# JelleAalbers/blueice

Hardware: AMD Instinct MI355X
Metric: likelihood evals/sec (and GB/s vs HBM peak), 4-src 5^3-anchor 100^3-bin model (higher is better)
Workload: dtype f64; 1 GPU; C2: 4 sources, 3 shape params (5^3 anchors), 100^3 bins; step = one batched call (one kernel launch) of 8 independent dense evaluations, each against its own dataset, in grid cells that share no anchor (no byte re-used), tensor replicated per GPU; device=gfx950:sramecc+:xnack-, gather=none (one process), backend_requested=rccl, backend_explicit=False, gather_kind=none (one process)

## Files before the change

blueice_amd/csrc/bi_context.h:

```cpp
#pragma once

struct bi_ctx;

constexpr int kThreads = 256;
constexpr int kBinsPerThread = 2;
constexpr int kTile = kThreads * kBinsPerThread;
constexpr int kMaxDim = 8;
constexpr int kMaxG = 16;

inline thread_local std::string g_create_error;

struct DevBuf {
    void* p = nullptr;
    size_t bytes = 0;
    struct bi_ctx* owner = nullptr;
    bool view = false;
};

struct bi_plan {
    int64_t P = 0;
    struct Class {
        int G = 0;
        int64_t n_items = 0;
        int nbx = 0;
// ... 42 lines not shown
    hipDeviceProp_t prop{};
    std::string err;

    bool model_ready = false, model_open = false;
    int d = 0, S = 0;
    int64_t B = 0, Bp = 0, A = 0;
    std::vector<int> n_anchor;
    std::vector<std::vector<double>> grid;
    std::vector<int64_t> astride;
    std::vector<int> eff_axes;
    int bb_source = -1;
    std::vector<int32_t> allow_neg;
    DevBuf ps, nm, nm_tot;
    std::vector<double> h_mus;
    std::vector<double> h_nm_tot;
    std::vector<char> anchor_set;

    int space_k = 0;
    std::vector<int32_t> space_n_edges;
    DevBuf space_edges;

    bool unbinned = false;
    double outlier = 0.0;
    bool ps_finite = true;
    bool data_ready = false;
    bool dense_counts = false;
    int64_t T = 0;
    DevBuf counts, lgsum;
    std::vector<double> h_lgsum;

    std::vector<double> h_rowsum;
    std::vector<double> h_rowmin;
    bool ps_nonneg = false;

    bool csr_ready = false, compact_ready = false;
    bool compact_sorted = false;
    DevBuf nz_idx, nz_n, nz_off, ps_c, cnt_c;
    DevBuf tm_entries, tm_off;
    int64_t nz_tile_epoch = -1;
    bool tm_ok = false;
    DevBuf tmm_entries, tmm_off;
    int64_t tmm_epoch = -1;
    bool tmm_ok = false;
    int tmm_width = 4;
    int64_t toy_points_pp = 0;
    int64_t toy_points_lanes = 0;
    int64_t toy_points_overlap = 0;
    hipStream_t stream2 = nullptr;
    hipEvent_t tp_ev[7] = {nullptr, nullptr, nullptr, nullptr, nullptr, nullptr, nullptr};
    int64_t n_toy_points_passes = 0;
    int64_t dot_tiled = 1;
    int64_t score_sorted = 1;
    DevBuf ev_perm;
    bool ev_sorted = false;
    int64_t toy_fast_call = 7;
    DevBuf toy_blocks_done;
    bool toy_blocks_done_zeroed = false;
    unsigned long long toy_seq = 0;
    int64_t n_toy_polled = 0;
    int64_t dot_entry16 = 1;
    int tm_width = 4;
    int64_t dot_blocks_per_cu = 0;
    int64_t dot_lanes = 0;
    int64_t toy_events = 1;
    int64_t last_toy_method = 0;
    std::vector<int64_t> h_nz_off;
    std::vector<int64_t> h_c_off, h_cnt_off;
    std::vector<int64_t> h_c_np;
    std::vector<double> h_Tz;

    DevBuf slot_dev, slot_partial, slot_pflags, slot_counter;
    DevBuf mail, mail_flags;
    void* pack_host = nullptr;
    void* bounce_host = nullptr;
    size_t pack_host_bytes = 0;
    DevBuf pack_dev;
    void* plan_host = nullptr;
    unsigned long long plan_seq = 0;
    void* slot_host = nullptr;
    size_t slot_host_bytes = 0;
    unsigned long long slot_seq = 0;
    int64_t single_ns[3] = {0, 0, 0};
    int64_t single_calls = 0;
    int pending = 0;
    unsigned long long pending_seq = 0;
    double pending_ll = 0.0;
    int32_t pending_status = 0;

    DevBuf pt_grid, pt_mus, pt_coff, pt_allow, pt_c_off, pt_cnt_off, pt_c_np, pt_Tz, pt_rowsum, pt_rowmin, pt_nm_tot;
    int64_t plan_tables_epoch = -1;
    bool plan_tables_sparse = false;
    int64_t n_valid_launches = 0;
    int64_t n_scan_launches = 0;
    int64_t last_scan_nslots = 0, last_scan_resident = 0, last_valid_nslots = 0;
    int64_t grad_mfma = 1;
    int64_t grad_mfma_min = 2048;
    int64_t grad_slices = 0;
    int64_t n_grad_mfma_launches = 0;
    int64_t scan_xcd = 1;
    int64_t scan_share_slow = 1;
    int64_t plan_count_sort = 1;
    int64_t plan_tables = 1;
    int64_t scan_chunk = 1;
    int64_t scan_waves_per_cu = 0;
    int64_t keep_rows = -1;
    int64_t last_single_cell = -1, last_single_ds = -1;
    int64_t poll_result = 1;
    int64_t tile_chunks = 8;
    int64_t scan_min_items = 4;
    int64_t toy_offset = 0;
    int64_t scan_cb = 0;
    int64_t bb_exact = 2;
    int64_t n_bb_exact = 0;
    int64_t scan_sparse_max_items = (int64_t)1 << 40;
    int64_t scan_split = 1;
    int64_t sparse_at_upload = 1;
    int64_t scan_mfma = 1;
    int64_t scan_pow = 1;
    DevBuf ps_sorted, cnt_sorted;
    int64_t sorted_epoch = -1;
    bool sorted_ok = false;
    int64_t n_sorted_scans = 0;
    int64_t mail_timeout_ms = 2000;
    int64_t debug_skip_post = -1, debug_late_post = -1;
    int64_t n_mail_resets = 0;
    std::vector<void*> user_allocs;
    int64_t bb_max_group = 8;
    int64_t scan_bb = 1;
    int64_t scan_bb_min = 64;
    int64_t n_bb_scan_launches = 0;
    int64_t device_plan_min = 512;

    DevBuf sim_coords, sim_source;
    int sim_k = 0;
    int64_t sim_n = -1;

    DevBuf scratch, scratch2, logmu;

    std::vector<DevBuf> cache;
    size_t cache_bytes = 0;

    int64_t epoch = 0;

    int64_t blocks_per_cu = 8;
    int64_t max_group = kMaxG;
    int64_t xcd_affine = 1;
    int64_t fuse_max_blocks = (int64_t)1 << 20;
    int64_t single_blocks_per_cu = 4;
    int64_t fuse_finish = 1;
    int64_t single_kernel = 1;
    int64_t nt_loads = 2;
    int64_t sparse = 1;
    int64_t compact_budget = (int64_t)16 << 30;

    bool profiling = false;
    std::vector<std::pair<hipEvent_t, hipEvent_t>> ev_pool;
    size_t ev_used = 0;
    int64_t prof_launches = 0;
    double prof_ms = 0.0;
};

namespace {

int fail(bi_ctx* c, int code, const char* fmt, ...) {
    char buf[512];
    va_list ap;
    va_start(ap, fmt);
    vsnprintf(buf, sizeof buf, fmt, ap);
    va_end(ap);
    if (c) c->err = buf; else g_create_error = buf;
    return code;
}

#define HIP_TRY(c, expr)                                                                          \
    do {                                                                                          \
        hipError_t e_ = (expr);                                                                   \
        if (e_ != hipSuccess)                                                                     \
            return fail((c), BI_ERR_HIP, "%s failed: %s (%s:%d)", #expr, hipGetErrorString(e_), __FILE__, __LINE__); \
    } while (0)

constexpr size_t kCacheMaxBuf = (size_t)1 << 30;
constexpr size_t kCacheMaxTotal = (size_t)4 << 30;
constexpr size_t kCacheMaxEntries = 256;

void dev_free(DevBuf& b) {
    if (b.p && !b.view) {
        bi_ctx* c = b.owner;
        if (c && b.bytes <= kCacheMaxBuf && c->cache.size() < kCacheMaxEntries && c->cache_bytes + b.bytes <= kCacheMaxTotal) {
            c->cache.push_back(b);
            c->cache_bytes += b.bytes;
        } else {
            (void)hipFree(b.p);
        }
    }
    b.p = nullptr;
    b.bytes = 0;
    b.view = false;
}

void drop_recycle_cache(bi_ctx* c) {
    (void)hipGetLastError();
    for (auto& q : c->cache) (void)hipFree(q.p);
    c->cache.clear();
    c->cache_bytes = 0;
}

int dev_alloc(bi_ctx* c, DevBuf& b, size_t bytes) {
    if (b.p && b.bytes >= bytes) return BI_OK;
    if (b.p) dev_free(b);
    if (bytes == 0) bytes = 16;
    if (bytes <= kCacheMaxBuf) {
        size_t best = (size_t)-1;
        for (size_t i = 0; i < c->cache.size(); ++i)
            if (c->cache[i].bytes >= bytes && c->cache[i].bytes <= 4 * bytes + 4096 &&
                (best == (size_t)-1 || c->cache[i].bytes < c->cache[best].bytes))
                best = i;
        if (best != (size_t)-1) {
            b = c->cache[best];
            c->cache_bytes -= b.bytes;
            c->cache[best] = c->cache.back();
            c->cache.pop_back();
            return BI_OK;
        }
    }
    hipError_t e = hipMalloc(&b.p, bytes);
    if (e != hipSuccess) {
        drop_recycle_cache(c);
        e = hipMalloc(&b.p, bytes);
    }
    if (e != hipSuccess) {
        b.p = nullptr;
        return fail(c, BI_ERR_NOMEM, "hipMalloc(%zu bytes) failed: %s", bytes, hipGetErrorString(e));
    }
    b.bytes = bytes;
    b.owner = c;
    return BI_OK;
}

template <class T>
int dev_upload(bi_ctx* c, DevBuf& b, const std::vector<T>& h) {
    int rc = dev_alloc(c, b, h.size() * sizeof(T));
    if (rc) return rc;
    if (!h.empty()) HIP_TRY(c, hipMemcpyAsync(b.p, h.data(), h.size() * sizeof(T), hipMemcpyHostToDevice, c->stream));
    return BI_OK;
}

struct PackedUpload {
    std::vector<size_t> off;
    size_t in_bytes = 0, out_off = 0;
    char* dev_base = nullptr;
    char* host_base = nullptr;
    template <typename T>
    const T* dev(size_t i) const { return reinterpret_cast<const T*>(dev_base + off[i]); }
    void* host_out() const { return host_base + out_off; }
};

inline int packed_upload(bi_ctx* c, const std::vector<std::pair<const void*, size_t>>& parts, size_t out_bytes, PackedUpload& pu,
                         DevBuf* slab = nullptr) {
    pu.off.clear();
    size_t total = 0;
    for (const auto& part : parts) {
        pu.off.push_back(total);
        total += (part.second + 63) / 64 * 64;
    }
    pu.in_bytes = total;
    pu.out_off = total;
    const size_t need = total + (out_bytes + 63) / 64 * 64 + 64;
    if (c->pack_host_bytes < need) {
        if (c->pack_host) { HIP_TRY(c, hipStreamSynchronize(c->stream)); HIP_TRY(c, hipHostFree(c->pack_host)); c->pack_host = nullptr; c->pack_host_bytes = 0; }
        const size_t grow = std::max<size_t>(2 * need, 65536);
        HIP_TRY(c, hipHostMalloc(&c->pack_host, grow, hipHostMallocDefault));
        c->pack_host_bytes = grow;
    }
    DevBuf& dst = slab ? *slab : c->pack_dev;
    int rc = dev_alloc(c, dst, std::max<size_t>(total, 64));
    if (rc) return rc;
    pu.host_base = (char*)c->pack_host;
    pu.dev_base = (char*)dst.p;
    for (size_t i = 0; i < parts.size(); ++i)
        if (parts[i].second) memcpy(pu.host_base + pu.off[i], parts[i].first, parts[i].second);
    if (total) HIP_TRY(c, hipMemcpyAsync(pu.dev_base, pu.host_base, total, hipMemcpyHostToDevice, c->stream));
    return BI_OK;
}

void free_plan_buffers(bi_plan* p) {
    for (auto& k : p->classes) {
        dev_free(k.rowoff); dev_free(k.coef); dev_free(k.aux); dev_free(k.item_cnt); dev_free(k.item_tiles);
        dev_free(k.perm); dev_free(k.slot_lg); dev_free(k.partial); dev_free(k.pflags); dev_free(k.rowoff_full);
    }
    dev_free(p->bad_idx); dev_free(p->nan_idx); dev_free(p->out); dev_free(p->status); dev_free(p->grp_first); dev_free(p->grp_items);
    dev_free(p->slab); dev_free(p->bad); dev_free(p->sorted_idx); dev_free(p->keep_z); dev_free(p->keep_rs);
}

}
```

blueice_amd/csrc/bi_k_misc.h:

```cpp
#pragma once

namespace {

__global__ void k_selftest_log(const double* __restrict__ x, int64_t n, double* __restrict__ out) {
    log_table_load();
    const int64_t i = (int64_t)blockIdx.x * blockDim.x + threadIdx.x;
    if (i < n) out[i] = bin_log(x[i]);
}

template <bool NT>
__global__ __launch_bounds__(kThreads) void k_read_sum(const double* __restrict__ p, int64_t n2, double* __restrict__ sink) {
    double s = 0.0;
    const int64_t stride = (int64_t)gridDim.x * kThreads;
    int64_t i = (int64_t)blockIdx.x * kThreads + threadIdx.x;
    for (; i + 7 * stride < n2; i += 8 * stride) {
        double2 v[8];
#pragma unroll
        for (int u = 0; u < 8; ++u) v[u] = stream_load<NT>(p + 2 * (i + u * stride));
#pragma unroll
        for (int u = 0; u < 8; ++u) s += v[u].x + v[u].y;
    }
    for (; i < n2; i += stride) s += p[2 * i] + p[2 * i + 1];
    if (s == 0.123456789) sink[0] = s;
}
// ... 275 lines not shown
    const double* __restrict__ r = rows + (int64_t)blockIdx.x * Bp;
    double s = 0.0, mn = __builtin_inf(), bad = 0.0;
    {
        double s4[4] = {0.0, 0.0, 0.0, 0.0};
        int64_t b = threadIdx.x;
        for (; b + 3 * kThreads < B; b += 4 * kThreads) {
            double v[4];
#pragma unroll
            for (int k = 0; k < 4; ++k) v[k] = r[b + k * kThreads];
#pragma unroll
            for (int k = 0; k < 4; ++k) {
                s4[k] += v[k];
                mn = fmin(mn, v[k]);
                if (!(fabs(v[k]) < __builtin_inf())) bad = 1.0;
            }
        }
        for (; b < B; b += kThreads) {
            const double v = r[b];
            s4[0] += v;
            mn = fmin(mn, v);
            if (!(fabs(v) < __builtin_inf())) bad = 1.0;
        }
        s = (s4[0] + s4[1]) + (s4[2] + s4[3]);
    }
    __shared__ double sh[3][kThreads / 64];
    s = wave_sum(s);
    bad = wave_sum(bad);
#pragma unroll
    for (int off = 32; off > 0; off >>= 1) mn = fmin(mn, __shfl_down(mn, off, 64));
    if ((threadIdx.x & 63) == 0) { sh[0][threadIdx.x >> 6] = s; sh[1][threadIdx.x >> 6] = mn; sh[2][threadIdx.x >> 6] = bad; }
    __syncthreads();
    if (threadIdx.x == 0) {
        double t = sh[0][0], m = sh[1][0], f = sh[2][0];
        for (int w = 1; w < kThreads / 64; ++w) { t += sh[0][w]; m = fmin(m, sh[1][w]); f += sh[2][w]; }
        out[(int64_t)blockIdx.x * 3 + 0] = t;
        out[(int64_t)blockIdx.x * 3 + 1] = m;
        out[(int64_t)blockIdx.x * 3 + 2] = f;
    }
}

constexpr int kNzPerThread = 8;
constexpr int kNzChunk = kThreads * kNzPerThread;

__device__ __forceinline__ bool is_nz(double n) { return n != 0.0; }

__global__ __launch_bounds__(kThreads) void k_nz_count(const double* __restrict__ counts, int64_t B, int64_t Bp,
                                                       int32_t* __restrict__ cnt, int nchunks) {
    const double* __restrict__ c = counts + (int64_t)blockIdx.y * Bp;
    const int64_t b0 = (int64_t)blockIdx.x * kNzChunk + threadIdx.x * kNzPerThread;
    int k = 0;
#pragma unroll
    for (int j = 0; j < kNzPerThread; ++j)
        if (b0 + j < B && is_nz(c[b0 + j])) ++k;
    __shared__ int sh[kThreads / 64];
#pragma unroll
    for (int off = 32; off > 0; off >>= 1) k += __shfl_down(k, off, 64);
    if ((threadIdx.x & 63) == 0) sh[threadIdx.x >> 6] = k;
    __syncthreads();
    if (threadIdx.x == 0) cnt[(int64_t)blockIdx.y * nchunks + blockIdx.x] = sh[0] + sh[1] + sh[2] + sh[3];
}

__global__ __launch_bounds__(kThreads) void k_nz_scatter(const double* __restrict__ counts, int64_t B, int64_t Bp,
                                                         const int64_t* __restrict__ chunk_off, int nchunks,
                                                         int32_t* __restrict__ nz_idx, double* __restrict__ nz_n) {
    const double* __restrict__ c = counts + (int64_t)blockIdx.y * Bp;
    const int64_t b0 = (int64_t)blockIdx.x * kNzChunk + threadIdx.x * kNzPerThread;
    double v[kNzPerThread];
    int k = 0;
#pragma unroll
    for (int j = 0; j < kNzPerThread; ++j) {
        v[j] = (b0 + j < B) ? c[b0 + j] : 0.0;
        if (is_nz(v[j])) ++k;
    }
    const int lane = threadIdx.x & 63, wave = threadIdx.x >> 6;
    int incl = k;
#pragma unroll
    for (int off = 1; off < 64; off <<= 1) {
        const int t = __shfl_up(incl, off, 64);
        if (lane >= off) incl += t;
    }
    __shared__ int sh[kThreads / 64];
    if (lane == 63) sh[wave] = incl;
    __syncthreads();
    int base = 0;
    for (int w = 0; w < wave; ++w) base += sh[w];
    int64_t pos = chunk_off[(int64_t)blockIdx.y * nchunks + blockIdx.x] + base + incl - k;
#pragma unroll
    for (int j = 0; j < kNzPerThread; ++j)
        if (is_nz(v[j])) {
            nz_idx[pos] = (int32_t)(b0 + j);
            nz_n[pos] = v[j];
            ++pos;
        }
}

__global__ __launch_bounds__(kThreads) void k_gather_rows(const double* __restrict__ rows, int64_t Bp,
                                                          const int32_t* __restrict__ idx, int64_t nnz, int64_t np,
                                                          double* __restrict__ out) {
    const int64_t j = (int64_t)blockIdx.x * kThreads + threadIdx.x;
    if (j >= np) return;
    const int64_t row = blockIdx.y;
    out[row * np + j] = j < nnz ? rows[row * Bp + idx[j]] : 0.0;
}

__global__ void k_pad_copy(const double* __restrict__ src, int64_t n, int64_t np, double* __restrict__ dst) {
    const int64_t j = (int64_t)blockIdx.x * blockDim.x + threadIdx.x;
    if (j < np) dst[j] = j < n ? src[j] : 0.0;
}

__global__ __launch_bounds__(kThreads) void k_dataset_dot_csr(const int32_t* __restrict__ nz_idx,
                                                              const double* __restrict__ nz_n,
                                                              const int64_t* __restrict__ nz_off,
                                                              const double* __restrict__ logmu, int64_t t0,
                                                              double* __restrict__ partial) {
    const int64_t t = t0 + blockIdx.x;
    const int64_t lo = nz_off[t], hi = nz_off[t + 1];
    double s = 0.0;
    for (int64_t j = lo + threadIdx.x; j < hi; j += kThreads) {
        const double n = nz_n[j];
        double term = n * logmu[nz_idx[j]];
        if (n != n) term = __builtin_nan("");
        else if (n < 0.0 || n != floor(n)) term = -__builtin_inf();
        s += term;
    }
    __shared__ double sh[kThreads / 64];
    s = wave_sum(s);
    if ((threadIdx.x & 63) == 0) sh[threadIdx.x >> 6] = s;
    __syncthreads();
    if (threadIdx.x == 0) {
        double r = sh[0];
        for (int w = 1; w < kThreads / 64; ++w) r += sh[w];
        partial[blockIdx.x] = r;
    }
}

constexpr int kDotTile = 8192;

__global__ __launch_bounds__(kThreads) void k_csr_tile_offsets(const int32_t* __restrict__ nz_idx, const int64_t* __restrict__ nz_off,
                                                               int n_tl, int32_t* __restrict__ tile_off ,
                                                               int tile_shift ) {
    const int64_t t = blockIdx.x;
    const int64_t lo = nz_off[t], hi = nz_off[t + 1];
    int32_t* __restrict__ dst = tile_off + t * (n_tl + 1);
    if (hi == lo) {
        for (int tl = threadIdx.x; tl <= n_tl; tl += kThreads) dst[tl] = 0;
        return;
    }
    for (int64_t j = lo + threadIdx.x; j < hi; j += kThreads) {
        const int cur = nz_idx[j] >> tile_shift;
        const int prev = j > lo ? nz_idx[j - 1] >> tile_shift : -1;
        for (int tl = prev + 1; tl <= cur; ++tl) dst[tl] = (int32_t)(j - lo);
        if (j == hi - 1)
            for (int tl = cur + 1; tl <= n_tl; ++tl) dst[tl] = (int32_t)(hi - lo);
    }
}

__device__ __forceinline__ double row16_sum(double v) {
#define BI_ROR_ADD(N)                                                                                              \
    do {                                                                                                           \
        const unsigned long long u = __double_as_longlong(v);                                                      \
        const unsigned lo = __builtin_amdgcn_update_dpp(0, (int)(unsigned)u, 0x120 + N, 0xF, 0xF, true);           \
        const unsigned hi = __builtin_amdgcn_update_dpp(0, (int)(unsigned)(u >> 32), 0x120 + N, 0xF, 0xF, true);   \
        v += __longlong_as_double(((unsigned long long)hi << 32) | lo);                                            \
    } while (0)
    BI_ROR_ADD(8);
    BI_ROR_ADD(4);
    BI_ROR_ADD(2);
    BI_ROR_ADD(1);
#undef BI_ROR_ADD
    return v;
}

constexpr uint32_t kTmPadEntry = (uint32_t)kDotTile << 3;
__global__ void k_tm_counts(const int32_t* __restrict__ tile_off, int64_t T, int n_tl, int64_t* __restrict__ cnt ,
                            int group ) {
    const int64_t i = (int64_t)blockIdx.x * blockDim.x + threadIdx.x;
    if (i > (int64_t)n_tl * T) return;
    if (i == (int64_t)n_tl * T) { cnt[i] = 0; return; }
    const int64_t tl = i / T, t = i % T;
    const int32_t* __restrict__ o = tile_off + t * (n_tl + 1) + tl;
    cnt[i] = (o[1] - o[0] + group - 1) & ~(group - 1);
}

template <typename ENTRY>
__global__ __launch_bounds__(kThreads) void k_tm_scatter(const int32_t* __restrict__ nz_idx, const double* __restrict__ nz_n,
                                                         const int64_t* __restrict__ nz_off, const int32_t* __restrict__ tile_off,
                                                         int64_t T, int n_tl, const int64_t* __restrict__ tm_off,
                                                         ENTRY* __restrict__ tm_entries, int* __restrict__ bad, int tile_shift) {
    const int64_t t = blockIdx.x;
    const int64_t lo = nz_off[t], hi = nz_off[t + 1];
    const int32_t* __restrict__ o = tile_off + t * (n_tl + 1);
    bool any_bad = false;
    for (int64_t j = lo + threadIdx.x; j < hi; j += kThreads) {
        const int idx = nz_idx[j];
        const double n = nz_n[j];
        const int tl = idx >> tile_shift;
        if constexpr (sizeof(ENTRY) == 2) {
            if (!(n >= 1.0 && n <= 7.0 && n == floor(n))) any_bad = true;
            tm_entries[tm_off[(int64_t)tl * T + t] + (j - lo - o[tl])] = (ENTRY)(((uint32_t)(idx - (tl << tile_shift)) << 3) | ((uint32_t)n & 7u));
        } else {
            if (!(n >= 1.0 && n < 32768.0 && n == floor(n))) any_bad = true;
            tm_entries[tm_off[(int64_t)tl * T + t] + (j - lo - o[tl])] = ((uint32_t)(idx - (tl << tile_shift)) << 3) | ((uint32_t)n << 17);
        }
    }
    if (any_bad) atomicOr(bad, 1);
}

typedef uint32_t bi_uint4 __attribute__((ext_vector_type(4)));
constexpr int kDotThreads = 1024;
#ifndef BI_DOT_DEPTH
#define BI_DOT_DEPTH 2
#endif
constexpr int kDotPad = 64 * 2 + 16;

template <int L>
__device__ __forceinline__ double row_group_sum(double v) {
#define BI_DPP_ADD(CTRL)                                                                                           \
    do {                                                                                                           \
        const unsigned long long u = __double_as_longlong(v);                                                      \
        const unsigned lo = __builtin_amdgcn_update_dpp(0, (int)(unsigned)u, CTRL, 0xF, 0xF, true);                \
        const unsigned hi = __builtin_amdgcn_update_dpp(0, (int)(unsigned)(u >> 32), CTRL, 0xF, 0xF, true);        \
        v += __longlong_as_double(((unsigned long long)hi << 32) | lo);                                            \
    } while (0)
    if constexpr (L == 16) {
        BI_DPP_ADD(0x120 + 8);
        BI_DPP_ADD(0x120 + 4);
        BI_DPP_ADD(0x120 + 2);
        BI_DPP_ADD(0x120 + 1);
    } else if constexpr (L == 8) {
        BI_DPP_ADD(0x141);
        BI_DPP_ADD(0xB1);
        BI_DPP_ADD(0x4E);
    } else if constexpr (L == 4) {
        BI_DPP_ADD(0xB1);
        BI_DPP_ADD(0x4E);
    } else {
        static_assert(L == 2, "groups of 2, 4, 8 or 16 lanes");
        BI_DPP_ADD(0xB1);
    }
#undef BI_DPP_ADD
    return v;
}

template <int L, int AHEAD, int W = 4>
__global__ __launch_bounds__(kDotThreads) void k_dataset_dot_tiled(const void* __restrict__ tm_entries_v,
                                                                   const int64_t* __restrict__ tm_off, int64_t T, int n_tl,
                                                                   const double* __restrict__ logmu, int64_t B, int64_t t0,
                                                                   int64_t n, double* __restrict__ partial ) {
    typedef typename std::conditional<W == 2, uint16_t, uint32_t>::type entry_t;
    constexpr int EPL = 16 / W;
    static_assert(EPL * L * AHEAD + 16 <= kDotPad, "the lists' padding must cover the read-ahead");
    const entry_t* __restrict__ tm_entries = static_cast<const entry_t*>(tm_entries_v);
    __shared__ double s_mu[kDotTile + 1];
    const int tl = blockIdx.x;
    const int64_t bin0 = (int64_t)tl * kDotTile;
    const int row = threadIdx.x / L, gl = threadIdx.x % L;
    const int per = (int)((n + gridDim.y - 1) / gridDim.y);
    const int c0u = (int)blockIdx.y * per, c1 = min((int)n, c0u + per);
    const int c0 = min(c0u, (int)n - 1);
    const int64_t* __restrict__ off = tm_off + (int64_t)tl * T + t0;
    const int64_t base = off[c0];
    const entry_t* __restrict__ ent = tm_entries + base;
    const uint32_t* __restrict__ off32 = reinterpret_cast<const uint32_t*>(off);
    const uint32_t base32 = (uint32_t)base;
    constexpr int kStep = kDotThreads / L, kAhead = AHEAD, kDepth = BI_DOT_DEPTH, kRing = 2 * (kDepth + 1);
    const int q_last = max(c0, c1 - 1);
    auto load_offsets = [&](int q, uint32_t& ra, uint32_t& rb) {
        const int qc = min(q, q_last);
        ra = off32[2 * qc];
        rb = off32[2 * qc + 2];
    };
    auto load_entries = [&](uint32_t ra, bi_uint4 (&e)[kAhead]) {
        const entry_t* __restrict__ p = ent + (int)(ra - base32) + EPL * gl;
#pragma unroll
        for (int k = 0; k < kAhead; ++k) __builtin_memcpy(&e[k], p + EPL * L * k, 16);
    };
    bi_uint4 E[kDepth + 1][kAhead];
    uint32_t RA[kRing], RB[kRing];
    const int q0 = c0 + row;
#pragma unroll
    for (int u = 0; u < 2 * kDepth; ++u) load_offsets(q0 + u * kStep, RA[u], RB[u]);
    {
        double v[kDotTile / kDotThreads];
#pragma unroll
        for (int k = 0; k < kDotTile / kDotThreads; ++k) v[k] = logmu[min(bin0 + threadIdx.x + k * kDotThreads, B - 1)];
#pragma unroll
        for (int k = 0; k < kDotTile / kDotThreads; ++k)
            s_mu[threadIdx.x + k * kDotThreads] = bin0 + threadIdx.x + k * kDotThreads < B ? v[k] : 0.0;
        if (threadIdx.x == 0) s_mu[kDotTile] = 0.0;
    }
#pragma unroll
    for (int u = 0; u < kDepth; ++u) load_entries(RA[u], E[u]);
    __syncthreads();
    if (c0u >= c1) return;
    const int n_iter = (c1 - c0 + kStep - 1) / kStep;
    for (int it = 0; it < n_iter; it += kRing) {
#pragma unroll
        for (int u = 0; u < kRing; ++u) {
            if (it + u < n_iter) {
                const int q = q0 + (it + u) * kStep;
                load_offsets(q + 2 * kDepth * kStep, RA[(u + 2 * kDepth) % kRing], RB[(u + 2 * kDepth) % kRing]);
                load_entries(RA[(u + kDepth) % kRing], E[(u + kDepth) % (kDepth + 1)]);
                __builtin_amdgcn_sched_barrier(0);
                const bi_uint4 (&e)[kAhead] = E[u % (kDepth + 1)];
                const int a = (int)(RA[u % kRing] - base32), b = (int)(RB[u % kRing] - base32);
                const int len = b - a - EPL * gl;
// ... 784 lines not shown
```

blueice_amd/csrc/bi_params.h:

```cpp
#pragma once

namespace {

enum : int { kParamRead = 1, kParamWrite = 2, kParamRW = 3 };

struct ParamDef {
    const char* name;
    int access;
    int64_t (*get)(bi_ctx*);
    int (*set)(bi_ctx*, int64_t);
};

#define BI_P_GET(expr) [](bi_ctx* c) -> int64_t { return (int64_t)(expr); }
#define BI_P_SET(stmt) [](bi_ctx* c, int64_t v) -> int { stmt; return BI_OK; }
#define BI_P_RANGE(lo, hi, field, what)                                                                           \
    [](bi_ctx* c, int64_t v) -> int {                                                                             \
        if (v < (lo) || v > (hi)) return fail(c, BI_ERR_INVALID, what);                                           \
        c->field = v;                                                                                             \
        return BI_OK;                                                                                             \
    }
#define BI_P_FLAG(field) BI_P_SET(c->field = v ? 1 : 0)
#define BI_P_RO(nm, expr) {nm, kParamRead, BI_P_GET(expr), nullptr}

const ParamDef kParams[] = {
    {"sparse", kParamRW, BI_P_GET(c->sparse), BI_P_RANGE(0, 2, sparse, "sparse: 0 = off, 1 = auto, 2 = whenever exact")},
    {"max_group", kParamRW, BI_P_GET(c->max_group),
     [](bi_ctx* c, int64_t v) -> int {
         if (v < 1 || v > kMaxG || (v & (v - 1))) return fail(c, BI_ERR_INVALID, "max_group must be a power of two in [1,%d]", kMaxG);
         c->max_group = v;
         return BI_OK;
     }},
    {"bb_max_group", kParamRW, BI_P_GET(c->bb_max_group), BI_P_SET(c->bb_max_group = v >= 16 ? 16 : (v >= 8 ? 8 : (v >= 4 ? 4 : (v >= 2 ? 2 : 1))))},
    {"blocks_per_cu", kParamRW, BI_P_GET(c->blocks_per_cu), BI_P_RANGE(1, 32, blocks_per_cu, "blocks_per_cu in [1,32]")},
    {"nt_loads", kParamRW, BI_P_GET(c->nt_loads), BI_P_RANGE(0, 2, nt_loads, "nt_loads: 0 = never, 1 = always, 2 = auto")},
    {"tile_chunks", kParamRW, BI_P_GET(c->tile_chunks), BI_P_SET(c->tile_chunks = v < 1 ? 1 : v)},
    {"single_kernel", kParamRW, BI_P_GET(c->single_kernel), BI_P_FLAG(single_kernel)},
    {"fuse_max_blocks", kParamRW, BI_P_GET(c->fuse_max_blocks), BI_P_SET(c->fuse_max_blocks = v)},
    {"single_blocks_per_cu", kParamRW, BI_P_GET(c->single_blocks_per_cu),
     BI_P_RANGE(1, 32, single_blocks_per_cu, "single_blocks_per_cu in [1,32]")},
    {"fuse_finish", kParamRW, BI_P_GET(c->fuse_finish), BI_P_FLAG(fuse_finish)},
    {"keep_rows", kParamRW, BI_P_GET(c->keep_rows), BI_P_SET(c->keep_rows = v < 0 ? -1 : v)},
    {"poll_result", kParamRW, BI_P_GET(c->poll_result), BI_P_FLAG(poll_result)},
    {"xcd_affine", kParamRW, BI_P_GET(c->xcd_affine), BI_P_FLAG(xcd_affine)},
    {"device_plan_min", kParamRW, BI_P_GET(c->device_plan_min), BI_P_SET(c->device_plan_min = v)},
    {"scan_mfma", kParamRW, BI_P_GET(c->scan_mfma), BI_P_FLAG(scan_mfma)},
    {"scan_min_items", kParamRW, BI_P_GET(c->scan_min_items), BI_P_SET(c->scan_min_items = v < 1 ? 1 : v)},
    {"scan_cb", kParamRW, BI_P_GET(c->scan_cb), BI_P_SET(c->scan_cb = (v == 2 || v == 4) ? v : 0)},
    {"scan_waves_per_cu", kParamRW, BI_P_GET(c->scan_waves_per_cu), BI_P_SET(c->scan_waves_per_cu = v < 0 ? 0 : v)},
    {"host_threads", kParamRW, [](bi_ctx*) -> int64_t { return host_threads(); },
     [](bi_ctx* c, int64_t v) -> int { if (v < 0 || v > 256) return fail(c, BI_ERR_INVALID, "host_threads in [0, 256] (0 = by the process's affinity, at most 16)"); host_threads_setting().store((int)v); return BI_OK; }},
    {"toy_points_pp", kParamRW, BI_P_GET(c->toy_points_pp),
     [](bi_ctx* c, int64_t v) -> int {
         if (v != 0 && v != 1 && v != 2 && v != 4) return fail(c, BI_ERR_INVALID, "toy_points_pp: 0 = by the batch, 1 = point by point, 2 or 4 points per pass");
         c->toy_points_pp = v;
         return BI_OK;
     }},
    {"toy_points_overlap", kParamRW, BI_P_GET(c->toy_points_overlap), BI_P_FLAG(toy_points_overlap)},
    {"toy_points_lanes", kParamRW, BI_P_GET(c->toy_points_lanes),
     [](bi_ctx* c, int64_t v) -> int {
         if (v != 0 && v != 2 && v != 4 && v != 8) return fail(c, BI_ERR_INVALID, "toy_points_lanes: 0 = default, or 2 / 4 / 8");
         c->toy_points_lanes = v;
         return BI_OK;
     }},
    {"grad_mfma", kParamRW, BI_P_GET(c->grad_mfma), BI_P_FLAG(grad_mfma)},
    {"grad_mfma_min", kParamRW, BI_P_GET(c->grad_mfma_min), BI_P_RANGE(1, (int64_t)1 << 40, grad_mfma_min, "grad_mfma_min >= 1")},
    {"grad_slices", kParamRW, BI_P_GET(c->grad_slices), BI_P_RANGE(0, 4096, grad_slices, "grad_slices in [0, 4096]")},
    {"scan_xcd", kParamRW, BI_P_GET(c->scan_xcd), BI_P_RANGE(0, 2, scan_xcd, "scan_xcd: 0 launch order, 1 contiguous ranges, 2 one XCD per group")},
    {"scan_share_slow", kParamRW, BI_P_GET(c->scan_share_slow), BI_P_FLAG(scan_share_slow)},
    {"scan_chunk", kParamRW, BI_P_GET(c->scan_chunk), BI_P_FLAG(scan_chunk)},
    {"plan_tables", kParamRW, BI_P_GET(c->plan_tables), BI_P_FLAG(plan_tables)},
    {"plan_count_sort", kParamRW, BI_P_GET(c->plan_count_sort), BI_P_FLAG(plan_count_sort)},
    {"scan_bb", kParamRW, BI_P_GET(c->scan_bb), BI_P_FLAG(scan_bb)},
    {"scan_bb_min", kParamRW, BI_P_GET(c->scan_bb_min), BI_P_RANGE(1, (int64_t)1 << 40, scan_bb_min, "scan_bb_min >= 1")},
    {"scan_sparse_max_items", kParamRW, BI_P_GET(c->scan_sparse_max_items), BI_P_SET(c->scan_sparse_max_items = v < 0 ? 0 : v)},
    {"scan_split", kParamRW, BI_P_GET(c->scan_split), BI_P_FLAG(scan_split)},
    {"scan_pow", kParamRW, BI_P_GET(c->scan_pow), BI_P_SET(c->scan_pow = v ? 1 : 0; c->sorted_epoch = -1)},
    {"bb_exact", kParamRW, BI_P_GET(c->bb_exact), BI_P_RANGE(0, 2, bb_exact, "bb_exact: 0 never, 1 always, 2 auto")},
    {"toy_events", kParamRW, BI_P_GET(c->toy_events), BI_P_FLAG(toy_events)},
    {"dot_tiled", kParamRW, BI_P_GET(c->dot_tiled), BI_P_FLAG(dot_tiled)},
    {"score_sorted", kParamRW, BI_P_GET(c->score_sorted), BI_P_FLAG(score_sorted)},
    {"toy_fast_call", kParamRW, BI_P_GET(c->toy_fast_call), BI_P_RANGE(0, 7, toy_fast_call, "toy_fast_call: bits 1 | 2 | 4")},
    {"dot_entry16", kParamRW, BI_P_GET(c->dot_entry16), [](bi_ctx* c, int64_t v) -> int { c->dot_entry16 = v ? 1 : 0; c->nz_tile_epoch = -1; c->tmm_epoch = -1; return BI_OK; }},
    {"dot_blocks_per_cu", kParamRW, BI_P_GET(c->dot_blocks_per_cu), BI_P_RANGE(0, 16, dot_blocks_per_cu, "dot_blocks_per_cu in [0, 16]")},
    {"dot_lanes", kParamRW, BI_P_GET(c->dot_lanes), BI_P_SET(c->dot_lanes = (v == 16 || v == 8 || v == 4) ? v : 0)},
    {"compact_budget", kParamRW, BI_P_GET(c->compact_budget), BI_P_SET(c->compact_budget = v)},
    {"toy_offset", kParamRW, BI_P_GET(c->toy_offset), BI_P_RANGE(0, INT64_MAX, toy_offset, "toy_offset >= 0")},
    {"mail_timeout_ms", kParamRW, BI_P_GET(c->mail_timeout_ms),
     BI_P_RANGE(1, 60000, mail_timeout_ms, "mail_timeout_ms in [1, 60000]")},
    {"single_timing_reset", kParamWrite, nullptr,
     BI_P_SET(c->single_ns[0] = c->single_ns[1] = c->single_ns[2] = 0; c->single_calls = 0; (void)v)},
    {"drop_recycle_cache", kParamWrite, nullptr, BI_P_SET((void)hipSetDevice(c->device); (void)hipStreamSynchronize(c->stream); drop_recycle_cache(c); (void)v)},
    {"debug_skip_post", kParamWrite, nullptr, BI_P_SET(c->debug_skip_post = v < 0 ? -1 : v)},
    {"debug_late_post", kParamWrite, nullptr, BI_P_SET(c->debug_late_post = v < 0 ? -1 : v)},
    BI_P_RO("tile_bins", kTile),
    BI_P_RO("padded_bins", c->Bp),
    BI_P_RO("n_scan_launches", c->n_scan_launches),
    BI_P_RO("n_toy_polled", c->n_toy_polled),
    BI_P_RO("n_toy_points_passes", c->n_toy_points_passes),
    BI_P_RO("n_bb_scan_launches", c->n_bb_scan_launches),
    BI_P_RO("tmm_entry_bytes", c->tmm_ok ? c->tmm_width : 0),
    BI_P_RO("tm_entry_bytes", c->tm_width),
    BI_P_RO("events_sorted", c->ev_sorted ? 1 : 0),
    BI_P_RO("n_grad_mfma_launches", c->n_grad_mfma_launches),
    BI_P_RO("n_valid_launches", c->n_valid_launches),
    BI_P_RO("n_sorted_scans", c->n_sorted_scans),
    BI_P_RO("n_bb_exact", c->n_bb_exact),
    BI_P_RO("n_mail_resets", c->n_mail_resets),
    BI_P_RO("csr_ready", (c->csr_ready && (c->sparse_at_upload != 0 || !c->dense_counts)) ? 1 : 0),
    BI_P_RO("compact_ready", (c->compact_ready && c->ps_nonneg && (c->sparse_at_upload != 0 || !c->dense_counts)) ? 1 : 0),
    BI_P_RO("split_ready", (c->compact_ready && c->dense_counts) ? 1 : 0),
    BI_P_RO("ps_nonneg", c->ps_nonneg ? 1 : 0),
    BI_P_RO("compact_sorted", (c->compact_ready && c->compact_sorted) ? 1 : 0),
    BI_P_RO("nnz_total", c->csr_ready ? c->h_nz_off.back() : -1),
    BI_P_RO("last_scan_nslots", c->last_scan_nslots),
    BI_P_RO("last_valid_nslots", c->last_valid_nslots),
    BI_P_RO("last_scan_resident", c->last_scan_resident),
    BI_P_RO("last_toy_method", c->last_toy_method),
    BI_P_RO("single_calls", c->single_calls),
    BI_P_RO("single_ns_host", c->single_ns[0]),
    BI_P_RO("single_ns_launch", c->single_ns[1]),
    BI_P_RO("single_ns_wait", c->single_ns[2]),
    BI_P_RO("user_allocations", (int64_t)c->user_allocs.size()),
    BI_P_RO("recycle_cache_bytes", (int64_t)c->cache_bytes),
};

#undef BI_P_GET
#undef BI_P_SET
#undef BI_P_RANGE
#undef BI_P_FLAG
#undef BI_P_RO

const ParamDef* find_param(const char* name) {
    for (const ParamDef& p : kParams)
        if (!strcmp(p.name, name)) return &p;
    return nullptr;
}

}
```

blueice_amd/csrc/bi_sparse.h:

```cpp
#pragma once

#include <rocprim/rocprim.hpp>

namespace {

int build_compact_templates(bi_ctx* c) {
    c->compact_ready = false;
    const int64_t T = c->T, Bp = c->Bp;
    int rc;
    hipError_t e;
    if (c->bb_source >= 0 || !c->ps_finite) return BI_OK;
    const int64_t rows = c->A * c->S;
    c->h_c_np.assign((size_t)T, 0);
    c->h_c_off.assign((size_t)T, 0);
    c->h_cnt_off.assign((size_t)T, 0);
    int64_t tot_ps = 0, tot_cnt = 0;
    for (int64_t t = 0; t < T; ++t) {
        const int64_t nnz = c->h_nz_off[(size_t)t + 1] - c->h_nz_off[(size_t)t];
        const int64_t np = std::max<int64_t>(kTile, (nnz + kTile - 1) / kTile * kTile);
        c->h_c_np[(size_t)t] = np;
        c->h_c_off[(size_t)t] = tot_ps;
        c->h_cnt_off[(size_t)t] = tot_cnt;
        tot_ps += rows * np;
        tot_cnt += np;
    }
    if ((tot_ps + tot_cnt) * (int64_t)sizeof(double) > c->compact_budget) return BI_OK;
    auto roomy = [&](DevBuf& b, size_t bytes) { return b.p && b.bytes >= bytes ? BI_OK : dev_alloc(c, b, bytes + bytes / 8); };
    if ((rc = roomy(c->ps_c, (size_t)tot_ps * sizeof(double))) || (rc = roomy(c->cnt_c, (size_t)tot_cnt * sizeof(double))) ||
        (rc = dev_alloc(c, c->scratch, (size_t)T * rows * sizeof(double))))
        return rc;
    c->h_Tz.assign((size_t)T * rows, 0.0);
    std::vector<double> tnz((size_t)T * rows);
    c->compact_sorted = false;
    const bool sort_by_count = c->scan_pow && T <= 64;
    DevBuf d_sidx, d_sn, d_tmp;
    auto drop = [&]() { dev_free(d_sidx); dev_free(d_sn); dev_free(d_tmp); };
    for (int64_t t = 0; t < T; ++t) {
        const int64_t lo = c->h_nz_off[(size_t)t], nnz = c->h_nz_off[(size_t)t + 1] - lo, np = c->h_c_np[(size_t)t];
        double* dst = (double*)c->ps_c.p + c->h_c_off[(size_t)t];
        const int32_t* idx = (const int32_t*)c->nz_idx.p + lo;
        const double* cnt = (const double*)c->nz_n.p + lo;
        if (sort_by_count && nnz > 1) {
            size_t tmp_bytes = 0;
            (void)prim_sort_pairs(nullptr, tmp_bytes, (const double*)nullptr, (double*)nullptr, (const int32_t*)nullptr,
                                            (int32_t*)nullptr, (size_t)nnz, 0u, 64u, c->stream);
            if ((rc = dev_alloc(c, d_sidx, (size_t)nnz * sizeof(int32_t))) || (rc = dev_alloc(c, d_sn, (size_t)nnz * sizeof(double))) ||
                (rc = dev_alloc(c, d_tmp, std::max<size_t>(tmp_bytes, 256)))) { drop(); return rc; }
            size_t tb = d_tmp.bytes;
            e = prim_sort_pairs(d_tmp.p, tb, cnt, (double*)d_sn.p, idx, (int32_t*)d_sidx.p, (size_t)nnz, 0u, 64u, c->stream);
            if (e != hipSuccess) { drop(); return fail(c, BI_ERR_HIP, "template compaction (sort by count): %s", hipGetErrorString(e)); }
            idx = (const int32_t*)d_sidx.p;
            cnt = (const double*)d_sn.p;
        }
        hipLaunchKernelGGL(k_gather_rows, dim3((unsigned)((np + kThreads - 1) / kThreads), (unsigned)rows), dim3(kThreads), 0,
                           c->stream, (const double*)c->ps.p, Bp, idx, nnz, np, dst);
        hipLaunchKernelGGL(k_pad_copy, dim3((unsigned)((np + 255) / 256)), dim3(256), 0, c->stream,
                           cnt, nnz, np, (double*)c->cnt_c.p + c->h_cnt_off[(size_t)t]);
        hipLaunchKernelGGL(k_row_total, dim3((unsigned)rows), dim3(kThreads), 0, c->stream, (const double*)dst, np, np,
                           (double*)c->scratch.p + t * rows);
        e = hipGetLastError();
        if (e != hipSuccess) { (void)hipStreamSynchronize(c->stream); drop(); return fail(c, BI_ERR_HIP, "template compaction: %s", hipGetErrorString(e)); }
    }
    e = hipMemcpyAsync(tnz.data(), c->scratch.p, tnz.size() * sizeof(double), hipMemcpyDeviceToHost, c->stream);
    if (e == hipSuccess) e = hipStreamSynchronize(c->stream);
    else (void)hipStreamSynchronize(c->stream);
    drop();
    if (e != hipSuccess) return fail(c, BI_ERR_HIP, "template compaction: %s", hipGetErrorString(e));
    for (int64_t t = 0; t < T; ++t)
        for (int64_t r = 0; r < rows; ++r) c->h_Tz[(size_t)(t * rows + r)] = c->h_rowsum[(size_t)r] - tnz[(size_t)(t * rows + r)];
    c->compact_sorted = sort_by_count;
    c->compact_ready = true;
    return BI_OK;
}

int build_sparse_forms(bi_ctx* c) {
    c->csr_ready = c->compact_ready = false;
    const int64_t T = c->T, B = c->B, Bp = c->Bp;
    const int nchunks = (int)((B + kNzChunk - 1) / kNzChunk);
    int rc;
    DevBuf d_cnt, d_off;
    auto cleanup = [&]() { dev_free(d_cnt); dev_free(d_off); };
    if ((rc = dev_alloc(c, d_cnt, (size_t)T * nchunks * sizeof(int32_t)))) return rc;
    const int64_t tchunk = 32768;
    for (int64_t t0 = 0; t0 < T; t0 += tchunk) {
        const int64_t n = std::min(tchunk, T - t0);
        hipLaunchKernelGGL(k_nz_count, dim3((unsigned)nchunks, (unsigned)n), dim3(kThreads), 0, c->stream,
                           (const double*)c->counts.p + t0 * Bp, B, Bp, (int32_t*)d_cnt.p + t0 * nchunks, nchunks);
    }
    std::vector<int32_t> h_cnt((size_t)T * nchunks);
    hipError_t e = hipGetLastError();
    if (e == hipSuccess) e = hipMemcpyAsync(h_cnt.data(), d_cnt.p, h_cnt.size() * sizeof(int32_t), hipMemcpyDeviceToHost, c->stream);
    if (e == hipSuccess) e = hipStreamSynchronize(c->stream);
    if (e != hipSuccess) { cleanup(); return fail(c, BI_ERR_HIP, "non-empty-bin count: %s", hipGetErrorString(e)); }
    std::vector<int64_t> h_off(h_cnt.size());
    c->h_nz_off.assign((size_t)T + 1, 0);
    int64_t run = 0;
    for (int64_t t = 0; t < T; ++t) {
        c->h_nz_off[(size_t)t] = run;
        for (int k = 0; k < nchunks; ++k) { h_off[(size_t)t * nchunks + k] = run; run += h_cnt[(size_t)t * nchunks + k]; }
    }
    c->h_nz_off[(size_t)T] = run;
    c->sparse_at_upload = c->sparse;
    if (run > T * B / 4 && c->sparse != 2) { cleanup(); return BI_OK; }
    if ((rc = dev_upload(c, d_off, h_off)) || (rc = dev_alloc(c, c->nz_idx, (size_t)std::max<int64_t>(run, 1) * sizeof(int32_t))) ||
        (rc = dev_alloc(c, c->nz_n, (size_t)std::max<int64_t>(run, 1) * sizeof(double))) || (rc = dev_upload(c, c->nz_off, c->h_nz_off))) {
        cleanup();
        return rc;
    }
    for (int64_t t0 = 0; t0 < T; t0 += tchunk) {
        const int64_t n = std::min(tchunk, T - t0);
        hipLaunchKernelGGL(k_nz_scatter, dim3((unsigned)nchunks, (unsigned)n), dim3(kThreads), 0, c->stream,
                           (const double*)c->counts.p + t0 * Bp, B, Bp, (const int64_t*)d_off.p + t0 * nchunks, nchunks,
                           (int32_t*)c->nz_idx.p, (double*)c->nz_n.p);
    }
    e = hipGetLastError();
    if (e == hipSuccess) e = hipStreamSynchronize(c->stream);
    cleanup();
    if (e != hipSuccess) return fail(c, BI_ERR_HIP, "non-empty-bin scatter: %s", hipGetErrorString(e));
    c->csr_ready = true;

    return build_compact_templates(c);
}

}
```

Measured before the change: 26110 evals/s.

## Batch sparse template compaction across all templates with tiled gather kernels

Replaces the per-template loop of compaction launches with a batched path. Offsets are tiled per template, then one gather kernel stages each row's bin tile in shared memory and scatters the non-empty bins to every template's compacted output. Batched kernels then do padding copy and row totals. This targets setup cost from many small launches; the per-evaluation likelihood kernels are unchanged. It adds complexity and a flag to fall back to the old path.

```diff
diff --git a/blueice_amd/csrc/bi_context.h b/blueice_amd/csrc/bi_context.h
--- a/blueice_amd/csrc/bi_context.h
+++ b/blueice_amd/csrc/bi_context.h
@@ -218,6 +218,8 @@
     int64_t nt_loads = 2;
     int64_t sparse = 1;
     int64_t compact_budget = (int64_t)16 << 30;
+    int64_t compact_batched = 1;
+    int64_t n_compact_batched = 0;
 
     bool profiling = false;
     std::vector<std::pair<hipEvent_t, hipEvent_t>> ev_pool;
diff --git a/blueice_amd/csrc/bi_k_misc.h b/blueice_amd/csrc/bi_k_misc.h
--- a/blueice_amd/csrc/bi_k_misc.h
+++ b/blueice_amd/csrc/bi_k_misc.h
@@ -451,6 +451,108 @@
         for (int tl = prev + 1; tl <= cur; ++tl) dst[tl] = (int32_t)(j - lo);
         if (j == hi - 1)
             for (int tl = cur + 1; tl <= n_tl; ++tl) dst[tl] = (int32_t)(hi - lo);
+    }
+}
+
+constexpr int kCompactThreads = 1024;
+constexpr int kCompactRuns = 4;
+static_assert(kDotTile == 1 << 13, "k_csr_tile_offsets is called with a shift of 13");
+
+__global__ __launch_bounds__(kCompactThreads) void k_gather_tiles(const double* __restrict__ rows, int64_t Bp,
+                                                                  const int32_t* __restrict__ nz_idx, const int64_t* __restrict__ nz_off,
+                                                                  int64_t nnz_all ,
+                                                                  const int32_t* __restrict__ tile_off , int n_tl, int64_t T,
+                                                                  const int64_t* __restrict__ c_off, const int64_t* __restrict__ c_np,
+                                                                  double* __restrict__ out) {
+    __shared__ double s_tile[kDotTile];
+    const int64_t row = blockIdx.x;
+    const int tl = blockIdx.y;
+    const int64_t bin0 = (int64_t)tl * kDotTile;
+    const double* __restrict__ src = rows + row * Bp + bin0;
+    {
+        const int n_in = (int)(Bp - bin0 < (int64_t)kDotTile ? Bp - bin0 : (int64_t)kDotTile);
+        constexpr int kPieces = kDotTile / 2 / kCompactThreads;
+        double2 v[kPieces];
+#pragma unroll
+        for (int k = 0; k < kPieces; ++k) {
+            const int i = 2 * ((int)threadIdx.x + k * kCompactThreads);
+            v[k] = i < n_in ? *reinterpret_cast<const double2*>(src + i) : make_double2(0.0, 0.0);
+        }
+#pragma unroll
+        for (int k = 0; k < kPieces; ++k) *reinterpret_cast<double2*>(s_tile + 2 * ((int)threadIdx.x + k * kCompactThreads)) = v[k];
+        __syncthreads();
+    }
+    const int lane = threadIdx.x & 63;
+    const int wave = __builtin_amdgcn_readfirstlane((int)threadIdx.x >> 6);
+    constexpr int kWaves = kCompactThreads / 64;
+    const bool pad = tl == n_tl - 1;
+    for (int64_t tb = (int64_t)wave * kCompactRuns; tb < T; tb += (int64_t)kWaves * kCompactRuns) {
+        int a[kCompactRuns], b[kCompactRuns];
+        int64_t lo[kCompactRuns], nnz[kCompactRuns], np[kCompactRuns];
+        double* dst[kCompactRuns];
+        int32_t i0[kCompactRuns], i1[kCompactRuns];
+#pragma unroll
+        for (int u = 0; u < kCompactRuns; ++u) {
+            const int64_t t = tb + u < T ? tb + u : T - 1;
+            const int32_t* __restrict__ o = tile_off + t * (n_tl + 1) + tl;
+            lo[u] = nz_off[t];
+            nnz[u] = nz_off[t + 1] - lo[u];
+            np[u] = c_np[t];
+            dst[u] = out + c_off[t] + row * np[u];
+            a[u] = max(o[0], 0);
+            b[u] = tb + u < T ? (int)min((int64_t)o[1], nnz[u]) : a[u];
+        }
+#pragma unroll
+        for (int u = 0; u < kCompactRuns; ++u) {
+            i0[u] = nz_idx[min(lo[u] + a[u] + lane, nnz_all - 1)];
+            i1[u] = nz_idx[min(lo[u] + a[u] + 64 + lane, nnz_all - 1)];
+        }
+#pragma unroll
+        for (int u = 0; u < kCompactRuns; ++u) {
+            const int j0 = a[u] + lane, j1 = j0 + 64;
+            if (j0 < b[u]) dst[u][j0] = s_tile[i0[u] - (int)bin0];
+            if (j1 < b[u]) dst[u][j1] = s_tile[i1[u] - (int)bin0];
+            for (int j = j1 + 64; j < b[u]; j += 64) dst[u][j] = s_tile[nz_idx[lo[u] + j] - (int)bin0];
+            if (pad && tb + u < T)
+                for (int64_t j = nnz[u] + lane; j < np[u]; j += 64) dst[u][j] = 0.0;
+        }
+    }
+}
+
+__global__ void k_pad_copy_batched(const double* __restrict__ nz_n, const int64_t* __restrict__ nz_off,
+                                   const int64_t* __restrict__ cnt_off, const int64_t* __restrict__ c_np, int64_t t0,
+                                   double* __restrict__ cnt_c) {
+    const int64_t t = t0 + blockIdx.y;
+    const int64_t j = (int64_t)blockIdx.x * blockDim.x + threadIdx.x;
+    if (j >= c_np[t]) return;
+    const int64_t lo = nz_off[t], n = nz_off[t + 1] - lo;
+    cnt_c[cnt_off[t] + j] = j < n ? nz_n[lo + j] : 0.0;
+}
+
+__global__ __launch_bounds__(kThreads) void k_row_total_batched(const double* __restrict__ ps_c, const int64_t* __restrict__ c_off,
+                                                                const int64_t* __restrict__ c_np, int64_t t0, int64_t n_rows,
+                                                                double* __restrict__ out ) {
+    const int64_t t = t0 + blockIdx.y;
+    const int64_t np = c_np[t];
+    const double* __restrict__ r = ps_c + c_off[t] + (int64_t)blockIdx.x * np;
+    double s = 0.0;
+    int64_t b = threadIdx.x;
+    for (; b + 3 * kThreads < np; b += 4 * kThreads) {
+        double v[4];
+#pragma unroll
+        for (int k = 0; k < 4; ++k) v[k] = r[b + k * kThreads];
+#pragma unroll
+        for (int k = 0; k < 4; ++k) s += v[k];
+    }
+    for (; b < np; b += kThreads) s += r[b];
+    __shared__ double sh[kThreads / 64];
+    s = wave_sum(s);
+    if ((threadIdx.x & 63) == 0) sh[threadIdx.x >> 6] = s;
+    __syncthreads();
+    if (threadIdx.x == 0) {
+        double tot = sh[0];
+        for (int w = 1; w < kThreads / 64; ++w) tot += sh[w];
+        out[t * n_rows + blockIdx.x] = tot;
     }
 }
 
diff --git a/blueice_amd/csrc/bi_params.h b/blueice_amd/csrc/bi_params.h
--- a/blueice_amd/csrc/bi_params.h
+++ b/blueice_amd/csrc/bi_params.h
@@ -84,6 +84,7 @@
     {"dot_blocks_per_cu", kParamRW, BI_P_GET(c->dot_blocks_per_cu), BI_P_RANGE(0, 16, dot_blocks_per_cu, "dot_blocks_per_cu in [0, 16]")},
     {"dot_lanes", kParamRW, BI_P_GET(c->dot_lanes), BI_P_SET(c->dot_lanes = (v == 16 || v == 8 || v == 4) ? v : 0)},
     {"compact_budget", kParamRW, BI_P_GET(c->compact_budget), BI_P_SET(c->compact_budget = v)},
+    {"compact_batched", kParamRW, BI_P_GET(c->compact_batched), BI_P_FLAG(compact_batched)},
     {"toy_offset", kParamRW, BI_P_GET(c->toy_offset), BI_P_RANGE(0, INT64_MAX, toy_offset, "toy_offset >= 0")},
     {"mail_timeout_ms", kParamRW, BI_P_GET(c->mail_timeout_ms),
      BI_P_RANGE(1, 60000, mail_timeout_ms, "mail_timeout_ms in [1, 60000]")},
@@ -106,6 +107,7 @@
     BI_P_RO("n_sorted_scans", c->n_sorted_scans),
     BI_P_RO("n_bb_exact", c->n_bb_exact),
     BI_P_RO("n_mail_resets", c->n_mail_resets),
+    BI_P_RO("n_compact_batched", c->n_compact_batched),
     BI_P_RO("csr_ready", (c->csr_ready && (c->sparse_at_upload != 0 || !c->dense_counts)) ? 1 : 0),
     BI_P_RO("compact_ready", (c->compact_ready && c->ps_nonneg && (c->sparse_at_upload != 0 || !c->dense_counts)) ? 1 : 0),
     BI_P_RO("split_ready", (c->compact_ready && c->dense_counts) ? 1 : 0),
diff --git a/blueice_amd/csrc/bi_sparse.h b/blueice_amd/csrc/bi_sparse.h
--- a/blueice_amd/csrc/bi_sparse.h
+++ b/blueice_amd/csrc/bi_sparse.h
@@ -3,6 +3,42 @@
 #include <rocprim/rocprim.hpp>
 
 namespace {
+
+int compact_ensemble(bi_ctx* c, int64_t rows, int n_tl) {
+    const int64_t T = c->T;
+    const size_t tb = (size_t)T * sizeof(int64_t);
+    int rc;
+    DevBuf d_tab, d_tile;
+    PackedUpload pu;
+    if ((rc = packed_upload(c, {{c->h_c_off.data(), tb}, {c->h_cnt_off.data(), tb}, {c->h_c_np.data(), tb}}, 0, pu, &d_tab)) ||
+        (rc = dev_alloc(c, d_tile, (size_t)T * (n_tl + 1) * sizeof(int32_t)))) {
+        dev_free(d_tab); dev_free(d_tile);
+        return rc;
+    }
+    const int64_t* c_off = pu.dev<int64_t>(0);
+    const int64_t* cnt_off = pu.dev<int64_t>(1);
+    const int64_t* c_np = pu.dev<int64_t>(2);
+    const int64_t* nz_off = (const int64_t*)c->nz_off.p;
+    const int64_t max_np = *std::max_element(c->h_c_np.begin(), c->h_c_np.end());
+    hipLaunchKernelGGL(k_csr_tile_offsets, dim3((unsigned)T), dim3(kThreads), 0, c->stream, (const int32_t*)c->nz_idx.p, nz_off, n_tl,
+                       (int32_t*)d_tile.p, 13);
+    hipLaunchKernelGGL(k_gather_tiles, dim3((unsigned)rows, (unsigned)n_tl), dim3(kCompactThreads), 0, c->stream, (const double*)c->ps.p, c->Bp,
+                       (const int32_t*)c->nz_idx.p, nz_off, std::max<int64_t>(c->h_nz_off.back(), 1), (const int32_t*)d_tile.p, n_tl, T,
+                       c_off, c_np, (double*)c->ps_c.p);
+    const int64_t tchunk = 65535;
+    for (int64_t t0 = 0; t0 < T; t0 += tchunk) {
+        const unsigned n = (unsigned)std::min(tchunk, T - t0);
+        hipLaunchKernelGGL(k_pad_copy_batched, dim3((unsigned)((max_np + 255) / 256), n), dim3(256), 0, c->stream,
+                           (const double*)c->nz_n.p, nz_off, cnt_off, c_np, t0, (double*)c->cnt_c.p);
+        hipLaunchKernelGGL(k_row_total_batched, dim3((unsigned)rows, n), dim3(kThreads), 0, c->stream, (const double*)c->ps_c.p, c_off,
+                           c_np, t0, rows, (double*)c->scratch.p);
+    }
+    const hipError_t e = hipGetLastError();
+    dev_free(d_tab); dev_free(d_tile);
+    if (e != hipSuccess) { (void)hipStreamSynchronize(c->stream); return fail(c, BI_ERR_HIP, "template compaction (ensemble): %s", hipGetErrorString(e)); }
+    ++c->n_compact_batched;
+    return BI_OK;
+}
 
 int build_compact_templates(bi_ctx* c) {
     c->compact_ready = false;
@@ -35,7 +71,10 @@
     const bool sort_by_count = c->scan_pow && T <= 64;
     DevBuf d_sidx, d_sn, d_tmp;
     auto drop = [&]() { dev_free(d_sidx); dev_free(d_sn); dev_free(d_tmp); };
-    for (int64_t t = 0; t < T; ++t) {
+    const int64_t n_tl = (c->B + kDotTile - 1) / kDotTile;
+    const bool batched = c->compact_batched && !sort_by_count && n_tl <= 65535;
+    if (batched && (rc = compact_ensemble(c, rows, (int)n_tl))) return rc;
+    for (int64_t t = 0; t < T && !batched; ++t) {
         const int64_t lo = c->h_nz_off[(size_t)t], nnz = c->h_nz_off[(size_t)t + 1] - lo, np = c->h_c_np[(size_t)t];
         double* dst = (double*)c->ps_c.p + c->h_c_off[(size_t)t];
         const int32_t* idx = (const int32_t*)c->nz_idx.p + lo;
```

Result: slower. 25650 evals/s (-1.7%).
